# matsengrp/linearham

Hardware: AMD Instinct MI355X
Metric: phylo-HMM log-likelihood evals/sec (100-leaf x 400-site family) (higher is better)
Workload: dtype f64

## Files before the change

linearham_amd/csrc/lh_capi.hip:

```cpp
#include <algorithm>
#include <array>
#include <map>
#include <cstdio>
#include <cstring>
#include <functional>
#include <atomic>
#include <chrono>
#include <string>
#include <thread>
#include <utility>
#include <vector>

#include "lh_device.h"

namespace lh {
const DebugOptions& debug_options() {
  static const DebugOptions opts = [] {
    DebugOptions o;
    auto set = [](const char* name) { return std::getenv(name) != nullptr; };
    auto num = [](const char* name, int dflt) { const char* e = std::getenv(name); return e ? std::atoi(e) : dflt; };
    o.chunk = std::max(256, num("LH_CHUNK", o.chunk));
    o.host_sub = std::max(256, num("LH_HOST_SUB", o.host_sub));
    o.eval_split = std::min(8, std::max(0, num("LH_EVAL_SPLIT", o.eval_split)));
    o.k0_serial = set("LH_K0_SERIAL");
    o.eval_fwd_priority = std::min(1, num("LH_EVAL_FWD_PRIORITY", o.eval_fwd_priority));
    o.k2b_no_pair = set("LH_K2B_NO_PAIR");
    o.k2b_vd_single = set("LH_K2B_VD_SINGLE");
    o.k2b_dj_pair = set("LH_K2B_DJ_PAIR");
    o.sample_timing = set("LH_SAMPLE_TIMING");
    o.k4_no_save = set("LH_K4_NO_SAVE");
    o.k1_tile_cap = num("LH_K1_TILE_CAP", 0);
    o.k1_cxx_walk = set("LH_K1_CXX_WALK");
    o.k1_tables = set("LH_K1_TABLES");
    o.k1_stack = set("LH_K1_STACK");
    o.k1_no_tables = set("LH_K1_NO_TABLES");
    o.k1_segments = set("LH_K1_SEGMENTS");
    o.k1_seg_waves = num("LH_K1_SEG_WAVES", o.k1_seg_waves);
    o.k1_no_fuse = set("LH_K1_NO_FUSE");
    o.codon_blocks = std::max(1, num("LH_CODON_BLOCKS", o.codon_blocks));
    o.events_blocks = std::max(1, num("LH_EVENTS_BLOCKS", o.events_blocks));
    o.anc_out_mb = std::max(1, num("LH_ANC_OUT_MB", o.anc_out_mb));
    o.edge_out_mb = std::max(1, num("LH_EDGE_OUT_MB", o.edge_out_mb));
    o.anc_pairs = std::max(0, num("LH_ANC_PAIRS", o.anc_pairs));
    o.collect_hash_bits = std::min(64, std::max(1, num("LH_COLLECT_HASH_BITS", o.collect_hash_bits)));
    return o;
  }();
  return opts;
}
}

namespace {

thread_local std::string g_error;

int fail(const std::string& msg) {
  g_error = msg;
  return 1;
}

#define LH_HIP(expr)                                                                      \
  do {                                                                                    \
    hipError_t e_ = (expr);                                                               \
    if (e_ != hipSuccess)                                                                 \
      return fail(std::string(#expr) + ": " + hipGetErrorString(e_));                     \
  } while (0)

template <bool Pinned>
class Buffer {
 public:
  Buffer() = default;
  Buffer(const Buffer&) = delete;
  Buffer& operator=(const Buffer&) = delete;
  ~Buffer() { release(); }
  int ensure(size_t bytes) {
    bytes = std::max<size_t>(bytes, 64);
    if (bytes <= cap_) return 0;
    if (p_) {
      LH_HIP(hipDeviceSynchronize());
      release();
    }
    LH_HIP(Pinned ? hipHostMalloc(&p_, bytes, hipHostMallocDefault) : hipMalloc(&p_, bytes));
    cap_ = bytes;
    return 0;
  }
  template <typename T = void>
  T* get() const { return static_cast<T*>(p_); }

 private:
  void release() {
    if (p_) (void)(Pinned ? hipHostFree(p_) : hipFree(p_));
    p_ = nullptr;
    cap_ = 0;
  }
  void* p_ = nullptr;
  size_t cap_ = 0;
};
using DevBuf = Buffer<false>;
using PinnedBuf = Buffer<true>;

template <int Stages>
class KernelTimer {
 public:
  KernelTimer() = default;
  KernelTimer(const KernelTimer&) = delete;
  KernelTimer& operator=(const KernelTimer&) = delete;
  ~KernelTimer() {
    for (Events& es : done_) destroy(es);
    destroy(open_);
    destroy(done_spans_);
    destroy(open_spans_);
  }
  int begin(hipStream_t s) {
    destroy(open_);
    for (hipEvent_t& e : open_) LH_HIP(hipEventCreate(&e));
    return mark(0, s);
  }
  int mark(int k, hipStream_t s) {
    LH_HIP(hipEventRecord(open_[k], s));
    return 0;
  }
  int end(hipStream_t s) {
    if (mark(Stages, s)) return 1;
    done_.push_back(std::exchange(open_, Events{}));
    return 0;
  }
  void begin_spans() {
    destroy(open_);
    destroy(open_spans_);
  }
  int span_begin(int stage, hipStream_t s) {
    Span sp{stage, nullptr, nullptr};
    LH_HIP(hipEventCreate(&sp.a));
    open_spans_.push_back(sp);
    LH_HIP(hipEventCreate(&open_spans_.back().b));
    LH_HIP(hipEventRecord(sp.a, s));
    return 0;
  }
  int span_end(hipStream_t s) {
    LH_HIP(hipEventRecord(open_spans_.back().b, s));
    return 0;
  }
  void end_spans() {
    done_spans_.insert(done_spans_.end(), open_spans_.begin(), open_spans_.end());
    open_spans_.clear();
    ++span_groups_;
  }
  int read(double* ms, int64_t* launches) {
    double sum[Stages] = {};
    hipError_t e = hipSuccess;
    for (Span& sp : done_spans_) {
      if (e == hipSuccess) e = hipEventSynchronize(sp.b);
      float t = 0;
      if (e == hipSuccess) e = hipEventElapsedTime(&t, sp.a, sp.b);
      sum[sp.stage] += t;
    }
    destroy(done_spans_);
    for (Events& es : done_) {
      if (e == hipSuccess) e = hipEventSynchronize(es[Stages]);
      for (int k = 0; k < Stages && e == hipSuccess; ++k) {
        float t = 0;
        e = hipEventElapsedTime(&t, es[k], es[k + 1]);
        sum[k] += t;
      }
      destroy(es);
    }
    const int64_t n = (int64_t)done_.size() + std::exchange(span_groups_, 0);
    done_.clear();
    LH_HIP(e);
    if (ms) std::copy(sum, sum + Stages, ms);
    if (launches) *launches = n;
    return 0;
  }

 private:
  using Events = std::array<hipEvent_t, Stages + 1>;
  static void destroy(Events& es) {
    for (hipEvent_t& e : es)
// ... 3791 lines not shown
```

linearham_amd/csrc/lh_device.h:

```cpp
#pragma once
#include <hip/hip_runtime.h>
#include <stdint.h>

#include <functional>

#include "linearham_amd.h"

namespace lh {

constexpr double kScaleFactor = 0x1p256;
constexpr double kScaleThreshold = 0x1p-256;
constexpr double kLogScaleFactor = 177.445678223345993274;

template <class... P, class... A>
static inline void launch_lds(void (*kernel)(P...), dim3 grid, dim3 block, size_t lds, hipStream_t stream,
                              const A&... args) {
  if (lds > 64 * 1024)
    (void)hipFuncSetAttribute(reinterpret_cast<const void*>(kernel), hipFuncAttributeMaxDynamicSharedMemorySize, (int)lds);
  hipLaunchKernelGGL(kernel, grid, block, lds, stream, args...);
}

enum : int { OP_CHERRY = 0, OP_TIP_ACC = 1, OP_POP_ACC = 2, OP_PUSH_FLAG = 16, OP_RANK_SHIFT = 8 };

enum : int { W_CHERRY = 0, W_TIP_ACC = 1, W_POP = 2, W_CTIP = 3, W_CTAB_ACC = 4 };
// ... 209 lines not shown
  return b.anc + ((size_t)v * (b.T - 2) + (node - b.T)) * b.L;
}
__device__ inline const uint8_t* slot_row(const LineageBatch& b, int x) { return slot_row(b, x / (b.P + 1), x % (b.P + 1)); }
constexpr uint64_t kLineagePadHash = 0;
void launch_lineage(const LineageBatch& b, uint64_t* nt_hash, uint64_t* aa_hash, hipStream_t stream);

template <class Rows>
void launch_store_verify(const Rows& src, int K, const int32_t* ids, const uint8_t* store, uint8_t* flag,
                         hipStream_t stream);
template <class Rows>
void launch_store_append(const Rows& src, int K, int n_pairs, const int32_t* pairs, uint8_t* store, hipStream_t stream);
template <class Rows>
void launch_store_gather(const Rows& src, int n_out, const int32_t* slots, uint8_t* out, hipStream_t stream);

__device__ static inline void compute_pmatrix(const double* __restrict__ e, double tr, double P[4][4]) {
  double ex[4];
#pragma unroll
  for (int k = 1; k < 4; ++k) ex[k] = expm1(e[k] * tr);
#pragma unroll
  for (int i = 0; i < 4; ++i)
#pragma unroll
    for (int j = 0; j < 4; ++j) {
      double v = (i == j) ? 1.0 : 0.0;
#pragma unroll
      for (int k = 1; k < 4; ++k) v = fma(e[4 + i * 4 + k] * ex[k], e[20 + k * 4 + j], v);
      P[i][j] = fmax(v, 0.0);
    }
}


void launch_model_setup(int n, int R, const double* er, const double* pi, const double* alpha,
                        double* rates, double* eig, hipStream_t stream);

int launch_prune(const DevFamily& fam, int n, int R, int T, int max_depth, const int32_t* ops,
                 const double* brlen, const double* rates, const double* eig, const PruneWs& ws, const double* pi,
                 double* site_lik, int32_t* site_scal, hipStream_t stream, bool allow_fused = true,
                 bool test_every_op = false, const PruneFork* fork = nullptr);
const char* prune_last_form();
const char* prune_last_error();

void launch_gtr_setup(int n, const double* er, const double* pi, double* eig, hipStream_t stream);

int launch_asr(const DevFamily& fam, int n, int R, int T, const int32_t* ops, const double* brlen, const double* rates,
               const double* eig, const double* pi, const double* site_lik, const int32_t* site_scal,
               const uint8_t* naive, uint64_t seed, uint64_t sample0, double* clv, void* desc, uint8_t* anc,
               uint8_t* rate_choice, const int4* hdr , hipStream_t stream,
               int draws = 1);
size_t asr_desc_bytes(int T);
size_t asr_lds_bytes(int T, int L, int R, int n_prune);
size_t asr_slots(int L, int R);

struct AsrOp {
  int4 a, b;
};

void launch_asr_sched(int n, int T, const int32_t* ops, const int4* hdr, void* desc, hipStream_t stream);

struct AncWs {
  double* clv;
  double* part;
  double* tvec;
  double* rho;
  int32_t* chain;
  int32_t* plen;
  void* desc;
};
struct AncWsBytes {
  size_t clv, part, tvec, rho, chain;
  size_t total() const { return clv + part + tvec + rho + chain; }
};
AncWsBytes anc_ws_bytes(int T, int L, int R, int n_prune, int P);
size_t anc_lds_bytes(int T);
int launch_ancestral(const DevFamily& fam, int n, int R, int T, const int32_t* ops, const double* brlen, const double* rates,
                     const double* eig, const double* pi, const double* site_lik, const int32_t* site_scal,
                     const double* naive_prob, const int32_t* path, int P, const AncWs& ws, double* marg, double* rate_post,
                     const int4* hdr, int32_t* err_flag, hipStream_t stream);
void launch_site_base(int n, int L, size_t forward_size, const int32_t* off, const int32_t* idx, const double* post,
                      const double* loglik, double* site_base, hipStream_t stream);
void launch_ancestral_ends(int n, int P, int L, const int32_t* plen, const double* marg, const double* loglik, double* ends,
                           double* ll_used, hipStream_t stream);
void launch_ancestral_front(const DevFamily& fam, int n, int R, int T, const int32_t* ops, const double* pi,
                            const double* site_lik, const int32_t* site_scal, const double* naive_prob, const int32_t* path,
                            int P, const AncWs& ws, double* rate_post, const int4* hdr, int32_t* err_flag, hipStream_t stream);
size_t anc_lp(int n_prune);

void launch_rate_sum(int n, int R, int slots, size_t width, bool last_live, const int32_t* plen, const double* part,
                     double* out, hipStream_t stream);

struct SubWs {
  double* cc;
  double* ne;
  double* se;
  double* el;
  double* edge;
};
struct SubWsBytes {
  size_t cc, ne, se, el, edge;
  size_t total(bool with_edge) const { return cc + ne + se + el + (with_edge ? edge : 0); }
};
SubWsBytes sub_ws_bytes(int L, int R, int P);
size_t sub_lds_bytes(int T, int P);
struct SubOut {
  double *edge, *naive_edge, *chain_counts, *seed_edge, *edge_load, *rate_post;
};
int launch_substitutions(const DevFamily& fam, int n, int R, int T, const int32_t* ops, const double* brlen, const double* rates,
                         const double* eig, const double* pi, const double* site_lik, const int32_t* site_scal,
                         const double* naive_prob, const int32_t* path, int P, int seed_tip, const AncWs& ws, const SubWs& sws,
                         const SubOut& out, const int4* hdr, int32_t* err_flag, hipStream_t stream);

struct CondWsBytes {
  size_t part, table;
};
CondWsBytes cond_ws_bytes(int R, int n_prune);
int launch_ancestral_cond(const DevFamily& fam, int n, int R, int T, const int32_t* ops, const double* brlen,
                          const double* rates, const double* eig, const double* pi, const double* site_lik,
                          const int32_t* site_scal, const double* naive_prob, const int32_t* path, int P, int node,
                          const AncWs& ws, double* table, double* cond, const int4* hdr, int32_t* err_flag,
                          hipStream_t stream);
void launch_row_mask(int n, int C, const int32_t* plen, double* em, hipStream_t stream);
void launch_pair_emissions(const DevFamily& fam, int K, long long q0, int count, const uint8_t* seqs, const int32_t* col_site,
                           const uint8_t* col_base, const int32_t* plen, const double* em, const double* table, double* out,
                           hipStream_t stream);
void launch_pair_finish(int K, long long q0, int count, const double* pair_ll, const double* open_ll, const int32_t* plen,
                        double* log_cand, double* prob, hipStream_t stream);

struct LogEmRequest {
  const int32_t* cols = nullptr;
  int n = 0;
  double* out = nullptr;
};
void launch_forward(const DevFamily& fam, const DevFamily* fam_dev, int n, int R, const double* site_lik,
                    const int32_t* site_scal, const double* pi, const double* em_in, double* em_out, double* gem,
                    int32_t* gcnt, double* jem,
                    int32_t* jrs, double* dxf, int32_t* dxc, double* loglik, double* forward_out, int32_t* scaler_out,
                    bool extended, hipStream_t stream, const LogEmRequest& lem = LogEmRequest{});
size_t forward_lds_bytes(const DevFamily& fam);
const char* forward_last_form();
int forward_last_dj_samples();
int forward_last_dj_waves();

size_t viterbi_bp_bytes(const DevFamily& fam);
size_t viterbi_lds_bytes(const DevFamily& fam);
void launch_viterbi(const DevFamily& fam, const DevSampler* smp_dev, int n, const double* gem, const int32_t* gcnt,
                    const double* jem, const int32_t* jrs, const double* loglik, uint8_t* bp, int32_t* states,
                    double* log_path, bool extended, hipStream_t stream);
void launch_path_prior(const DevFamily& fam, const DevSampler* smp_dev, int K, const int32_t* states, double* log_prior,
                       int32_t* first_bad, hipStream_t stream);

struct DebugOptions {
  int chunk = 49152;
  int host_sub = 12288;
  int eval_split = 0;
  bool k0_serial = false;
  int eval_fwd_priority = -1;
  bool k2b_no_pair = false;
  bool k2b_vd_single = false;
  bool k2b_dj_pair = false;
  bool sample_timing = false;
  bool k4_no_save = false;
  int k1_tile_cap = 0;
  bool k1_cxx_walk = false;
  bool k1_tables = false;
  bool k1_stack = false;
  bool k1_no_tables = false;
  bool k1_segments = false;
  int k1_seg_waves = 4;
  bool k1_no_fuse = false;
  int codon_blocks = 2048;
  int events_blocks = 1024;
  int anc_out_mb = 4096;
  int edge_out_mb = 4096;
  int anc_pairs = 0;
  int collect_hash_bits = 64;
};
const DebugOptions& debug_options();

}
```

linearham_amd/csrc/lh_prune.hip:

```cpp
#include <cstdlib>

#include <cstdio>
#include <type_traits>

#include "lh_device.h"

namespace lh {

namespace {

thread_local char g_prune_form[64] = "";
thread_local char g_prune_error[256] = "";

#define LH_SLOT_COPY(dst, src)                       \
  _Pragma("unroll") for (int s_ = 0; s_ < S; ++s_) { \
    dst[s_][0] = src[s_][0];                         \
    dst[s_][1] = src[s_][1];                         \
    dst[s_][2] = src[s_][2];                         \
    dst[s_][3] = src[s_][3];                         \
  }
#define LH_PUSH_IF(d)                                   \
  if constexpr (kDepth > d) {                           \
    if (push_mask & (1u << d)) { LH_SLOT_COPY(st##d, a) } \
  }
// ... 554 lines not shown
          mat_list[rank] = (uint16_t)(2 * k);
          if (kind == OP_POP_ACC) mat_list[rank + 1] = (uint16_t)(2 * k + 1);
        }
      }
      __syncthreads();
      const int n_inner = T - 3;
      for (int it = rtid; it < n_inner + T; it += nthr) {
        if (it < n_inner) {
          const int code = mat_list[it], k = min(code >> 1, n_ops - 1);
          const int4 op = op_ptr[k];
          const int node = min(max((code & 1) ? op.y : op.z, 0), nodes - 1);
          compute_pmatrix(e, bl[node] * rt, P);
          double* o = pw + (size_t)k * 32 + (code & 1) * 16;
#pragma unroll
          for (int i = 0; i < 4; ++i)
#pragma unroll
            for (int q = 0; q < 4; ++q) o[i * 4 + q] = P[i][q];
        } else {
          const int j = it - n_inner;
          compute_pmatrix(e, bl[j] * rt, P);
          double* o = tiptab + j * 16;
#pragma unroll
          for (int i = 0; i < 4; ++i)
#pragma unroll
            for (int st = 0; st < 4; ++st) o[st * 4 + i] = P[i][st];
        }
      }
    } else {
    const int half = nthr >= 128 ? (nthr / 128) * 64 : 0;
    const bool do_ops = half == 0 || rtid < half;
    const bool do_tips = half == 0 || rtid >= half;
    if (do_ops) {
      const int stride = half ? half : nthr;
      for (int k = rtid; k < n_ops; k += stride) {
        const int4 op = op_ptr[k];
        const int kind = op.x & 15;
        if (kind == OP_CHERRY) continue;
        double* o = pw + (size_t)k * 32;
        compute_pmatrix(e, bl[op.z] * rt, P);
#pragma unroll
        for (int i = 0; i < 4; ++i)
#pragma unroll
          for (int q = 0; q < 4; ++q) o[i * 4 + q] = P[i][q];
        if (kind == OP_POP_ACC) {
          compute_pmatrix(e, bl[op.y] * rt, P);
#pragma unroll
          for (int i = 0; i < 4; ++i)
#pragma unroll
            for (int q = 0; q < 4; ++q) o[16 + i * 4 + q] = P[i][q];
        }
      }
    }
    if (do_tips) {
      const int stride = half ? nthr - half : nthr;
      for (int j = half ? rtid - half : rtid; j < (kSeg ? 1 : T); j += stride) {
        compute_pmatrix(e, bl[j] * rt, P);
        double* o = kSeg ? tiptab + 2 * kSegOps * 16 : tiptab + j * 16;
#pragma unroll
        for (int i = 0; i < 4; ++i)
#pragma unroll
          for (int st = 0; st < 4; ++st) o[st * 4 + i] = P[i][st];
      }
    }
    }
  }
  SegCtx seg{eig + (size_t)sample * 36, brlen + (size_t)sample * (2 * (size_t)T - 2),
             rates[(size_t)sample * R + rate], tiptab, rtid, nthr};
  if constexpr (kSeg) seg_fill(seg, op_ptr, n_ops, 0);
  asm volatile("s_waitcnt vmcnt(0)" ::: "memory");
  __threadfence_block();
  __syncthreads();

  const pmat_ptr pm = pmat_after_barrier(pmat_w + pm_off);
  const int lane = tid & 63;
  const int tile0 = blockIdx.x * tile;
  const int site_end = min(tile0 + tile, L);
  const double* __restrict__ p4 = pi + (size_t)sample * 4;
  double lik[2][5];
  int scl[2] = {0, 0};
  int site0, n_own;
  bool two_sites = false;
  if constexpr (kTwo) two_sites = wave < n2;
  if (two_sites) {
    site0 = tile0 + wave * 128 + lane;
    n_own = 2;
    if constexpr (kTwo)
      prune_wave<kDepth, 2, kN, kSeg>(site0, site_end, msa, L, n_ops, op_ptr, pm, tiptab, naive_tab, ones_off, p4, lik, scl, seg);
  } else {
    site0 = tile0 + n2 * 128 + (wave - n2) * 64 + lane;
    n_own = 1;
    double lik1[1][5];
    int scl1[1];
    prune_wave<kDepth, 1, kN, kSeg>(site0, site_end, msa, L, n_ops, op_ptr, pm, tiptab, naive_tab, ones_off, p4, lik1, scl1, seg);
#pragma unroll
    for (int b = 0; b < 5; ++b) lik[0][b] = lik1[0][b];
    scl[0] = scl1[0];
  }

  if constexpr (!kFused) {
    double* lik_out = site_lik + (((size_t)sample * R + rate) * 5) * (size_t)L;
    int32_t* scal_out = site_scal + ((size_t)sample * R + rate) * (size_t)L;
#pragma unroll
    for (int s = 0; s < 2; ++s) {
      const int site = site0 + 64 * s;
      if (s < n_own && site < site_end) {
#pragma unroll
        for (int b = 0; b < 5; ++b) lik_out[(size_t)b * L + site] = lik[s][b];
        scal_out[site] = scl[s];
      }
    }
  } else {
    const int pad = n2 * 128 + (wpr - n2) * 64;
    __syncthreads();
    double* X = reinterpret_cast<double*>(smem2);
    int* SC = reinterpret_cast<int*>(X + (size_t)R * 5 * pad);
#pragma unroll
    for (int s = 0; s < 2; ++s) {
      const int idx = site0 + 64 * s - tile0;
      if (s < n_own && idx < pad) {
#pragma unroll
        for (int b = 0; b < 5; ++b) X[((size_t)rate * 5 + b) * pad + idx] = lik[s][b];
        SC[rate * pad + idx] = scl[s];
      }
    }
    __syncthreads();
    const int n_tile = site_end - tile0;
    const double w = 1.0 / R;
    double* lik_out = site_lik + ((size_t)sample * 5) * (size_t)L;
    int32_t* scal_out = site_scal + (size_t)sample * (size_t)L;
    for (int j = tid; j < 5 * n_tile; j += blockDim.x) {
      const int b = j / n_tile, p = j - b * n_tile;
      int smin = 0x7fffffff;
      for (int r = 0; r < R; ++r) smin = min(smin, SC[r * pad + p]);
      double acc = 0.0;
      for (int r = 0; r < R; ++r) {
        double v = X[((size_t)r * 5 + b) * pad + p];
        const int d = SC[r * pad + p] - smin;
        for (int q = 0; q < d && v != 0.0; ++q) v *= kScaleThreshold;
        acc += w * v;
      }
      lik_out[(size_t)b * L + tile0 + p] = acc;
      if (b == 0) scal_out[tile0 + p] = smin;
    }
  }
}

__device__ __forceinline__ void matvec_v(const double (&p)[16], const double (&a)[4], double (&x)[4]) {
  x[0] = fma(p[3], a[3], fma(p[2], a[2], fma(p[1], a[1], p[0] * a[0])));
  x[1] = fma(p[7], a[3], fma(p[6], a[2], fma(p[5], a[1], p[4] * a[0])));
  x[2] = fma(p[11], a[3], fma(p[10], a[2], fma(p[9], a[1], p[8] * a[0])));
  x[3] = fma(p[15], a[3], fma(p[14], a[2], fma(p[13], a[1], p[12] * a[0])));
}

__global__ void __launch_bounds__(64) schedule_rewrite_kernel(int T, int max_depth, int tabs_stride, int use_tables,
                                                              const int32_t* __restrict__ ops, const double* __restrict__ brlen,
                                                              int2* __restrict__ wops, double* __restrict__ wlen,
                                                              int4* __restrict__ tabs, int4* __restrict__ hdr, int32_t* err_flag) {
  extern __shared__ int k0c_lds[];
  int* tnode = k0c_lds;
  int* lastpush = k0c_lds + tabs_stride;
  const int lane = threadIdx.x, smp = blockIdx.x;
  const int n_ops = T - 2, nodes = 2 * T - 2;
  const int4* __restrict__ og = reinterpret_cast<const int4*>(ops) + (size_t)smp * n_ops;
  int2* wo = wops + (size_t)smp * n_ops;
  int4* tl = tabs + (size_t)smp * tabs_stride;
  double* ml = wlen + (size_t)smp * n_ops;
  const double* __restrict__ bl = brlen + (size_t)smp * nodes;
  if (lane < 16) lastpush[lane] = -1;
  __syncthreads();
  auto tip_ok = [&](int v) { return v >= 1 && v < T; };
  auto inner_ok = [&](int v) { return v >= T && v < nodes; };
  auto plain = [](int x) { return x >= 0 && (x & 0xf0) == 0; };
  auto fold = [&](int j, const int4& c, const int4& nx) -> int {
    if (!use_tables || j + 1 >= n_ops || (c.x & 15) != OP_CHERRY || c.x < 0 || (c.x & 0xe0)) return 0;
    const bool push = (c.x & OP_PUSH_FLAG) != 0;
    const int nk = nx.x & 15;
    if (push && nk == OP_POP_ACC && plain(nx.x) && nx.w == c.w && inner_ok(nx.y) && inner_ok(nx.z)) return 1;
    if (nk == OP_TIP_ACC && plain(nx.x) && tip_ok(nx.y) && inner_ok(nx.z)) return 2;
    return 0;
  };
  auto scan = [&](int v) {
#pragma unroll
    for (int d = 1; d < 64; d <<= 1) {
      const int up = __shfl_up(v, d);
      if (lane >= d) v += up;
    }
    return v;
  };
  int c_bdepth = 0, c_wi = 0, c_wdepth = 0, c_mi = 0, c_ti = 0;
  bool bad = false;
  const int4 none = make_int4(15, 0, 0, 0);
  for (int k0 = 0; k0 < n_ops; k0 += 64) {
    const int k = k0 + lane;
    const bool in = k < n_ops;
    const int4 op = in ? og[k] : none;
    const int4 nx = (in && k + 1 < n_ops) ? og[k + 1] : none;
    const int4 pv = (in && k > 0) ? og[k - 1] : none;
    const int kind = op.x & 15;
    const bool push = (op.x & OP_PUSH_FLAG) != 0;
    const int f = in ? fold(k, op, nx) : 0;
    const bool consumed = in && k > 0 && fold(k - 1, pv, op) != 0;
    bool ok = op.x >= 0 && (op.x & 0xe0) == 0 && kind <= OP_POP_ACC;
    if (kind == OP_CHERRY) ok = ok && tip_ok(op.y) && tip_ok(op.z) && push == (k != 0);
    if (kind == OP_TIP_ACC) ok = ok && !push && k > 0 && tip_ok(op.y) && inner_ok(op.z);
    if (kind == OP_POP_ACC) ok = ok && !push && k > 0 && inner_ok(op.y) && inner_ok(op.z);
    const int db = !in || !ok ? 0 : push ? 1 : kind == OP_POP_ACC ? -1 : 0;
    const int s_db = scan(db);
    const int bdepth = c_bdepth + s_db - db;
    if (in && push && (op.w != bdepth || bdepth >= max_depth)) ok = false;
    if (in && kind == OP_POP_ACC && op.w != bdepth - 1) ok = false;
    const bool emit = in && ok && !consumed;
    const bool wpush = emit && push && f != 1;
    const bool wpop = emit && kind == OP_POP_ACC;
    const bool hasmat = wpush || (emit && (f == 1 || kind == OP_TIP_ACC || kind == OP_POP_ACC));
    const bool hastab = emit && f != 0;
    const int e1 = emit ? 1 : 0, dw = wpush ? 1 : wpop ? -1 : 0, m1 = hasmat ? 1 : 0, t1 = hastab ? 1 : 0;
    const int s_e1 = scan(e1), s_dw = scan(dw), s_m1 = scan(m1), s_t1 = scan(t1);
    const int wi = c_wi + s_e1 - e1, wdepth = c_wdepth + s_dw - dw, mi = c_mi + s_m1 - m1, ti = c_ti + s_t1 - t1;
    if (wpush && wdepth >= 16) ok = false;
    if (wpop && wdepth < 1) ok = false;
    if (hastab && ti >= tabs_stride) ok = false;
    if (hasmat && mi >= n_ops) ok = false;
    if (in && !ok) bad = true;
    int mypush = -1;
    for (int d = 0; d < max_depth; ++d) {
      int v = (wpush && ok && wdepth == d) ? mi : -1;
#pragma unroll
      for (int q = 1; q < 64; q <<= 1) {
        const int up = __shfl_up(v, q);
        if (lane >= q) v = max(v, up);
      }
      v = max(v, lastpush[d]);
      if (wpop && wdepth - 1 == d) mypush = v;
      const int last = __shfl(v, 63);
      __syncthreads();
      if (lane == 0) lastpush[d] = last;
      __syncthreads();
    }
    if (wpop && mypush < 0) {
      ok = false;
      bad = true;
    }
    if (emit && ok) {
      int2 w;
      if (f == 1) {
        w = make_int2(W_CTAB_ACC | WOP_MATRIX | WOP_HAS_B | (op.y << 16), op.z | (1 << 16));
        ml[mi] = bl[nx.y];
      } else if (kind == OP_CHERRY) {
        const int pushbits = wpush ? WOP_MATRIX | ((wdepth + 1) << WOP_PUSH_SHIFT) : 0;
        w = f == 2 ? make_int2(W_CTIP | pushbits | WOP_HAS_B | WOP_HAS_C | (op.y << 16), op.z | (nx.y << 16))
                   : make_int2(W_CHERRY | pushbits | WOP_HAS_B | (op.y << 16), op.z | (1 << 16));
      } else if (kind == OP_TIP_ACC) {
        w = make_int2(W_TIP_ACC | WOP_MATRIX | (op.y << 16), 1 | (1 << 16));
        ml[mi] = bl[op.z];
      } else {
        w = make_int2(W_POP | WOP_MATRIX | ((wdepth - 1) << WOP_POP_SHIFT) | (1 << 16), 1 | (1 << 16));
        ml[mypush] = bl[op.y];
        ml[mi] = bl[op.z];
      }
      wo[wi] = w;
      if (hastab) {
        tl[ti] = make_int4(op.y, op.z, nx.z, 0);
        tnode[ti] = nx.z;
      }
    }
    c_bdepth += __shfl(s_db, 63);
    c_wi += __shfl(s_e1, 63);
    c_wdepth += __shfl(s_dw, 63);
    c_mi += __shfl(s_m1, 63);
    c_ti += __shfl(s_t1, 63);
  }
  if (c_bdepth != 0 || c_wdepth != 0 || c_mi + c_ti > T - 3) bad = true;
  const bool any_bad = __builtin_amdgcn_ballot_w64(bad) != 0;
  if (lane == 0) {
    if (any_bad) {
      hdr[smp] = make_int4(0, 0, 0, 1);
      atomicOr(err_flag, 1);
    } else {
      hdr[smp] = make_int4(c_wi, c_mi, c_ti, 0);
    }
  }
  if (any_bad) return;
  __syncthreads();
  for (int c = lane; c < c_ti; c += 64) ml[c_mi + c] = bl[tnode[c]];
}

__global__ void __launch_bounds__(64) schedule_stack_check_kernel(int T, int slots, int check_ranks,
                                                                  const int32_t* __restrict__ ops, int4* __restrict__ hdr,
                                                                  int32_t* err_flag) {
  const int smp = blockIdx.x, lane = threadIdx.x;
  const int n_ops = T - 2, nodes = 2 * T - 2;
  const int4* __restrict__ o = reinterpret_cast<const int4*>(ops) + (size_t)smp * n_ops;
  int carry = 0, depth0 = 0;
  bool bad = false;
  for (int k0 = 0; k0 < n_ops; k0 += 64) {
    const int k = k0 + lane;
    const bool in = k < n_ops;
    const int4 op = in ? o[k] : make_int4(OP_CHERRY, 1, 1, 0);
    const int kind = op.x & 15, rank = op.x >> OP_RANK_SHIFT;
    const bool push = (op.x & OP_PUSH_FLAG) != 0;
    bool ok = op.x >= 0 && (op.x & 0xe0) == 0 && kind <= OP_POP_ACC;
    if (kind == OP_CHERRY) ok = ok && op.y >= 1 && op.y < T && op.z >= 1 && op.z < T && push == (k != 0);
    if (kind == OP_TIP_ACC) ok = ok && !push && k > 0 && op.y >= 1 && op.y < T && op.z >= T && op.z < nodes;
    if (kind == OP_POP_ACC) ok = ok && !push && k > 0 && op.y >= T && op.y < nodes && op.z >= T && op.z < nodes;
    if (push || kind == OP_POP_ACC) ok = ok && op.w >= 0 && op.w < slots;
    const int m = !in || !ok ? 0 : kind == OP_TIP_ACC ? 1 : kind == OP_POP_ACC ? 2 : 0;
    const int dl = !in || !ok ? 0 : push ? 1 : kind == OP_POP_ACC ? -1 : 0;
    int incl = m, dincl = dl;
#pragma unroll
    for (int d = 1; d < 64; d <<= 1) {
      const int up = __shfl_up(incl, d), dup = __shfl_up(dincl, d);
      if (lane >= d) incl += up, dincl += dup;
    }
    const int depth = depth0 + dincl - dl;
    if (in && push && op.w != depth) ok = false;
    if (in && kind == OP_POP_ACC && op.w != depth - 1) ok = false;
    if (check_ranks && in && kind != OP_CHERRY && rank != carry + incl - m) ok = false;
    if (in && !ok) bad = true;
    carry += __shfl(incl, 63);
    depth0 += __shfl(dincl, 63);
  }
  if (carry != T - 3 || depth0 != 0) bad = true;
  const bool any_bad = __builtin_amdgcn_ballot_w64(bad) != 0;
  if (lane == 0) {
    hdr[smp] = make_int4(0, 0, 0, any_bad ? 1 : 0);
    if (any_bad) atomicOr(err_flag, 1);
  }
}

struct PruneCtArgs {
  int n2, tile, R, wpr;
  int L, T, tabs_stride, pad_;
  const uint8_t* msa;
  const uint64_t* planes;
  const int2* wops;
  const double* wlen;
  const int4* tabs;
  const int4* hdr;
  const double* brlen;
  const double* rates;
  const double* eig;
  double* pmat_w;
  size_t rate_stride;
  const double* pi;
  double* site_lik;
  int32_t* site_scal;
};
typedef const PruneCtArgs __attribute__((address_space(4)))* ct_args_ptr;
typedef int __attribute__((ext_vector_type(4))) ct_int4;

__device__ __forceinline__ ct_args_ptr ct_args_again(ct_args_ptr p) {
  uint64_t v = reinterpret_cast<uint64_t>(p);
  asm volatile("; lh: kernel arguments at %0, read again from here" : "+s"(v));
  return (ct_args_ptr)v;
}
__device__ __forceinline__ ct_args_ptr ct_args() { return ct_args_again((ct_args_ptr)__builtin_amdgcn_kernarg_segment_ptr()); }

template <class T, class U>
__device__ __forceinline__ const T __attribute__((address_space(4)))* ct_ro(const U* p) {
  return (const T __attribute__((address_space(4)))*)reinterpret_cast<uint64_t>(p);
}

struct CtWave {
  int rate, wave, nthr, rtid;
};
constexpr int kCtFusedMaxWaves = 16;
constexpr size_t kCtFusedMaxLds = 80 * 1024;
static_assert(kCtFusedMaxWaves <= 16, "ct_wave counts at most 15 steps");
static_assert(53 * 1024 <= kCtFusedMaxLds, "the limit of fused workgroups of up to eight waves (launch_prune) lies within it");
static_assert(3 * (kCtFusedMaxLds / 128) < (1u << 21), "prune_body_ct: c / rem through v_rcp_f32 needs R * rem < 2^21");
template <bool kFused>
__device__ __forceinline__ int ct_block_threads(int R, int wpr) {
  return (kFused ? R : 1) * wpr * 64;
}
template <bool kFused>
__device__ __forceinline__ CtWave ct_wave(int tid, int wpr) {
  const int wave_all = __builtin_amdgcn_readfirstlane(tid >> 6);
  if constexpr (kFused) {
    int rate = 0, wave = wave_all;
    for (; wave >= wpr && rate < 15; ++rate) wave -= wpr;
    return CtWave{rate, wave, wpr * 64, tid - rate * wpr * 64};
  } else {
    return CtWave{(int)blockIdx.y, wave_all, wpr * 64, tid};
  }
}

template <int kDepth, bool kN, bool kFused, bool kAsm = false>
__device__ __forceinline__ void prune_body_ct() {
  extern __shared__ double2 smem2[];
  constexpr int SY = kN ? 5 : 4, E = SY * SY;
  constexpr int kS = 2;
  const int tid = threadIdx.x;
  const int sample = blockIdx.z;
  const ct_args_ptr a0 = ct_args();
  const CtWave g = ct_wave<kFused>(tid, a0->wpr);
  const int rate = g.rate, wave = g.wave, nthr = g.nthr, rtid = g.rtid;
  {
    const ct_args_ptr a = a0;
    const int T = a->T, R = a->R;
    const int n_w = ct_ro<int>(a->hdr)[(size_t)sample * 4];
    if (kN && tid < 4) reinterpret_cast<double*>(smem2)[(kFused ? R : 1) * T * 16 + tid] = 1.0;
    const WalkOp* wops = a->wops + (size_t)sample * (T - 2);
    WalkOp* desc = reinterpret_cast<WalkOp*>(reinterpret_cast<double*>(smem2) + (size_t)(kFused ? R : 1) * T * 16 + (kN ? 4 : 0));
    for (int i = tid; i < n_w; i += ct_block_threads<kFused>(R, a->wpr))
      desc[i] = *reinterpret_cast<const WalkOp*>(reinterpret_cast<const char*>(wops) + (unsigned)i * 8u);
  }

  int4 tcell = make_int4(1, 1, 0, 0);
  double pcq[16];
  {
    const ct_args_ptr a = a0;
    const int T = a->T, R = a->R, n_ops = T - 2;
    const int n_mat = ct_ro<int>(a->hdr)[(size_t)sample * 4 + 1], n_tab = ct_ro<int>(a->hdr)[(size_t)sample * 4 + 2];
    const size_t rate_stride = a->rate_stride;
    const int n_q = min(n_tab, nthr >> 2);
    const bool in_quad = (rtid >> 2) < n_q;
    const bool pc_lane = (rtid & 3) == 0 && in_quad;
    if (in_quad) tcell = (a->tabs + (size_t)sample * a->tabs_stride)[rtid >> 2];
    const double* bl = a->brlen + (size_t)sample * (2 * (size_t)T - 2);
    const double* wl = a->wlen + (size_t)sample * n_ops;
    char* pw_s = reinterpret_cast<char*>(a->pmat_w + (size_t)sample * R * rate_stride);
    const unsigned rate_bytes = (unsigned)rate_stride * 8u;
    const int n_rest = n_tab - n_q;
// ... 204 lines not shown
    for (int s = 0; s < kS; ++s) {
      const int site = site0 + 64 * s;
      if (s < n_own && site < site_end) {
#pragma unroll
        for (int q = 0; q < 5; ++q) lik_out[(size_t)q * L_b + site] = lik[s][q];
        scal_out[site] = scl[s];
      }
    }
  } else {
    const int pad = n2_b * (64 * kS) + (b->wpr - n2_b) * 64;
    __syncthreads();
    double* X = reinterpret_cast<double*>(smem2);
    int* SC = reinterpret_cast<int*>(X + (size_t)R_b * 5 * pad);
#pragma unroll
    for (int s = 0; s < kS; ++s) {
      const int idx = site0 + 64 * s - tile0;
      if (s < n_own && idx < pad) {
#pragma unroll
        for (int q = 0; q < 5; ++q) X[((size_t)rate_b * 5 + q) * pad + idx] = lik[s][q];
        SC[rate_b * pad + idx] = scl[s];
      }
    }
    __syncthreads();
    const int n_tile = site_end - tile0;
    const double w = 1.0 / R_b;
    double* lik_out = b->site_lik + ((size_t)sample * 5) * (size_t)L_b;
    int32_t* scal_out = b->site_scal + (size_t)sample * (size_t)L_b;
    for (int p = tid_b; p < n_tile; p += ct_block_threads<kFused>(R_b, b->wpr)) {
      int smin = 0x7fffffff;
      for (int r = 0; r < R_b; ++r) smin = min(smin, SC[r * pad + p]);
      double acc[5] = {0.0, 0.0, 0.0, 0.0, 0.0};
      for (int r = 0; r < R_b; ++r) {
        const int d = SC[r * pad + p] - smin;
#pragma unroll
        for (int q = 0; q < 5; ++q) {
          double v = X[((size_t)r * 5 + q) * pad + p];
          for (int k = 0; k < d && v != 0.0; ++k) v *= kScaleThreshold;
          acc[q] += w * v;
        }
      }
#pragma unroll
      for (int q = 0; q < 5; ++q) lik_out[(size_t)q * L_b + tile0 + p] = acc[q];
      scal_out[tile0 + p] = smin;
    }
  }
}

#define LH_PRUNE_CT_KERNEL(NAME, WAVES)                                                              \
  template <int kDepth, bool kN, bool kFused, bool kAsm>                                             \
  __global__ void __launch_bounds__(1024) __attribute__((amdgpu_waves_per_eu(WAVES, WAVES))) NAME(   \
      const PruneCtArgs args ) {                                         \
    prune_body_ct<kDepth, kN, kFused, kAsm>();                                                       \
  }
LH_PRUNE_CT_KERNEL(prune_kernel_ct6, 6)
LH_PRUNE_CT_KERNEL(prune_kernel_ct5, 5)
LH_PRUNE_CT_KERNEL(prune_kernel_ct4, 4)
#undef LH_PRUNE_CT_KERNEL
#define LH_PRUNE_PARAMS                                                                                     \
  int n_samples, int n2, int tile, int R, int wpr, const uint8_t *__restrict__ msa, int L, int T, int n_ops, \
      const int32_t *__restrict__ ops, const int4 *__restrict__ hdr, int32_t *err_flag,                     \
      const double *__restrict__ brlen, const double *__restrict__ rates, const double *__restrict__ eig,  \
      double *pmat_w, size_t rate_stride, const double *__restrict__ pi,                                   \
      double *__restrict__ site_lik, int32_t *__restrict__ site_scal
#define LH_PRUNE_ARGS \
  n2, tile, R, wpr, msa, L, T, n_ops, ops, hdr, err_flag, brlen, rates, eig, pmat_w, rate_stride, pi, site_lik, site_scal
#define LH_PRUNE_SAMPLES(BODY) BODY((int)blockIdx.z, LH_PRUNE_ARGS);

#define LH_PRUNE_KERNEL(NAME, WAVES)                                                                 \
  template <int kDepth, bool kN>                                                                     \
  __global__ void __launch_bounds__(1024) __attribute__((amdgpu_waves_per_eu(WAVES, WAVES))) NAME(   \
      LH_PRUNE_PARAMS) {                                                                             \
    LH_PRUNE_SAMPLES((prune_body<kDepth, true, kN, true>))                                           \
  }
LH_PRUNE_KERNEL(prune_kernel_w6, 6)
LH_PRUNE_KERNEL(prune_kernel_w5, 5)
LH_PRUNE_KERNEL(prune_kernel_w4, 4)
#undef LH_PRUNE_KERNEL

template <int kDepth, bool kN>
__global__ void __launch_bounds__(512) __attribute__((amdgpu_waves_per_eu(5, 5))) prune_kernel_seg(LH_PRUNE_PARAMS) {
  LH_PRUNE_SAMPLES((prune_body<kDepth, true, kN, false, true>))
}
template <int kDepth, bool kN>
__global__ void __launch_bounds__(512) __attribute__((amdgpu_waves_per_eu(4, 4))) prune_kernel_seg4(LH_PRUNE_PARAMS) {
  LH_PRUNE_SAMPLES((prune_body<kDepth, true, kN, false, true>))
}

PruneWsSizes prune_ws_sizes(int T, bool mixed_n) {
  PruneWsSizes z;
  z.tabs_per_sample = (size_t)std::max((T - 1) / 2, 1);
  const size_t e = mixed_n ? 25 : 16;
  z.scratch_doubles_per_rate = std::max((size_t)std::max(T - 3, 0) * 16 + z.tabs_per_sample * e * 4, (size_t)std::max(T - 2, 1) * 32);
  return z;
}

int launch_prune(const DevFamily& fam, int n, int R, int T, int max_depth, const int32_t* ops,
                 const double* brlen, const double* rates, const double* eig, const PruneWs& ws, const double* pi,
                 double* site_lik, int32_t* site_scal, hipStream_t stream, bool allow_fused, bool test_every_op,
                 const PruneFork* fork) {
  hipStream_t sched = fork ? fork->sched : stream;
  auto joined = [&]() {
    if (!fork || fork->join() == 0) return true;
    snprintf(g_prune_error, sizeof(g_prune_error), "K1: the schedule kernel's stream could not be joined");
    return false;
  };
  const int L = fam.n_prune;
  const PruneWsSizes sizes = prune_ws_sizes(T, fam.msa_mixed_n != 0);
  if (L == 0) {
    hipLaunchKernelGGL(schedule_stack_check_kernel, dim3(n), dim3(64), 0, sched, T, std::max(max_depth, 1), 0, ops, ws.hdr, ws.err_flag);
    return joined() ? R : -1;
  }
  double* pmat = ws.scratch;
  const size_t rate_stride = sizes.scratch_doubles_per_rate;
  const DebugOptions& dbg = debug_options();
  const int cap_env = dbg.k1_tile_cap;
  const int cap = cap_env >= 64 ? std::min(cap_env, 1024) : 1024;
  const int tiles = (L + cap - 1) / cap;
  const int tile = tiles == 1 ? L : (((L + tiles - 1) / tiles + 127) & ~127);
  int n2 = tile / 128, n1;
  {
    const int rem = tile - 128 * n2;
    if (rem > 64) {
      ++n2;
      n1 = 0;
    } else {
      n1 = rem > 0 ? 1 : 0;
    }
  }
  const int wpr = n2 + n1;
  const size_t tip_bytes = (size_t)T * 16 * sizeof(double);
  const size_t pad = (size_t)n2 * 128 + (size_t)n1 * 64;
  const size_t tail_bytes = (((size_t)std::max(T - 2, 1) * sizeof(int2)) + 31) & ~(size_t)15;
  const bool mixed = fam.msa_mixed_n != 0;
  const size_t ones_bytes = mixed ? 32 : 0;
  const size_t fused_lds = std::max((size_t)R * tip_bytes + ones_bytes + tail_bytes, (size_t)R * pad * (5 * sizeof(double) + sizeof(int)));
  const bool fused = allow_fused && !dbg.k1_no_fuse && !dbg.k1_segments &&
                     ((R * wpr <= 8 && fused_lds <= 53 * 1024) ||
                      (R * wpr > 8 && R * wpr <= kCtFusedMaxWaves && fused_lds <= kCtFusedMaxLds));
  const bool big = !fused && ((160 * 1024 / tip_bytes) * wpr / 4 < 5 || dbg.k1_segments);
  const bool tables_hook = dbg.k1_tables || dbg.k1_no_tables;
  const bool use_asm = !dbg.k1_cxx_walk && !test_every_op;
  const bool stack_fused = fused && max_depth <= 4 && dbg.k1_stack && !tables_hook;
  const bool seg = big && max_depth <= 4 && !tables_hook;
  const size_t seg_bytes = (size_t)(2 * kSegOps + 1) * 16 * sizeof(double) + ones_bytes;
  size_t lds = fused ? fused_lds : seg ? seg_bytes : tip_bytes + ones_bytes + tail_bytes;
  if (lds > 160 * 1024) {
    snprintf(g_prune_error, sizeof(g_prune_error),
             "K1: a tree of %d tips with stack depth %d needs %zu bytes of LDS in the cherry-table form (160 KB per CU)", T, max_depth, lds);
    return -1;
  }
  if (stack_fused || seg) {
    hipLaunchKernelGGL(schedule_stack_check_kernel, dim3(n), dim3(64), 0, sched, T, stack_fused && max_depth <= 3 ? 3 : 4,
                       stack_fused ? 1 : 0, ops, ws.hdr, ws.err_flag);
  } else {
    hipLaunchKernelGGL(schedule_rewrite_kernel, dim3(n), dim3(64), (sizes.tabs_per_sample + 16) * sizeof(int), sched, T, max_depth,
                       (int)sizes.tabs_per_sample, dbg.k1_no_tables ? 0 : 1, ops, brlen, ws.wops, ws.wlen, ws.tabs, ws.hdr, ws.err_flag);
  }
  if (!joined()) return -1;
  const int wg_waves = fused ? R * wpr : wpr;
  dim3 grid(tiles, fused ? 1 : R, n), block(64 * wg_waves);
  const int n_ops = T - 2;
  hipError_t attr_rc = hipSuccess;
#define LH_LAUNCH_K(K, NAME)                                                                                     \
  {                                                                                                              \
    if (lds > 64 * 1024)                                                                                         \
      attr_rc = hipFuncSetAttribute(reinterpret_cast<const void*>(K), hipFuncAttributeMaxDynamicSharedMemorySize, (int)lds); \
    snprintf(g_prune_form, sizeof(g_prune_form), "%s", NAME);                                                    \
    if (attr_rc == hipSuccess)                                                                                   \
      hipLaunchKernelGGL(K, grid, block, lds, stream, n, n2, tile, R, wpr, fam.msa, L, T, n_ops, ops, ws.hdr, ws.err_flag, \
                         brlen, rates, eig, pmat, rate_stride, pi, site_lik, site_scal);                        \
  }
#define LH_LAUNCH_CT(K, NAME)                                                                                    \
  {                                                                                                              \
    if (lds > 64 * 1024)                                                                                         \
      attr_rc = hipFuncSetAttribute(reinterpret_cast<const void*>(K), hipFuncAttributeMaxDynamicSharedMemorySize, (int)lds); \
    snprintf(g_prune_form, sizeof(g_prune_form), "%s", NAME);                                                    \
    if (attr_rc == hipSuccess) hipLaunchKernelGGL(K, grid, block, lds, stream, ct_args);                        \
  }
  PruneCtArgs ct_args = {};
  ct_args.n2 = n2, ct_args.tile = tile, ct_args.R = R, ct_args.wpr = wpr;
  ct_args.L = L, ct_args.T = T, ct_args.tabs_stride = (int)sizes.tabs_per_sample;
  ct_args.msa = fam.msa, ct_args.planes = fam.msa_planes;
  ct_args.wops = ws.wops, ct_args.wlen = ws.wlen, ct_args.tabs = ws.tabs, ct_args.hdr = ws.hdr;
  ct_args.brlen = brlen, ct_args.rates = rates, ct_args.eig = eig;
  ct_args.pmat_w = pmat, ct_args.rate_stride = rate_stride;
  ct_args.pi = pi, ct_args.site_lik = site_lik, ct_args.site_scal = site_scal;
  const int lds_waves = lds == 0 ? 8 : (int)((160 * 1024 / lds) * wg_waves / 4);
  if (stack_fused) {
#define LH_LAUNCH_STACK(D, N)                                                          \
  {                                                                                    \
    if (lds_waves >= 6 && D == 3)                                                      \
      LH_LAUNCH_K((prune_kernel_w6<D, N>), "w6<" #D "," #N ">")                        \
    else if (lds_waves >= 5)                                                           \
      LH_LAUNCH_K((prune_kernel_w5<D, N>), "w5<" #D "," #N ">")                        \
    else                                                                               \
      LH_LAUNCH_K((prune_kernel_w4<D, N>), "w4<" #D "," #N ">")                        \
  }
    if (max_depth <= 3 && !mixed)
      LH_LAUNCH_STACK(3, false)
    else if (max_depth <= 3)
      LH_LAUNCH_STACK(3, true)
    else if (!mixed)
      LH_LAUNCH_STACK(4, false)
    else
      LH_LAUNCH_STACK(4, true)
#undef LH_LAUNCH_STACK
  } else if (seg) {
    if (dbg.k1_seg_waves == 4) {
      if (mixed)
        LH_LAUNCH_K((prune_kernel_seg4<4, true>), "seg4<4,true>")
      else
        LH_LAUNCH_K((prune_kernel_seg4<4, false>), "seg4<4,false>")
    } else {
      if (mixed)
        LH_LAUNCH_K((prune_kernel_seg<4, true>), "seg5<4,true>")
      else
        LH_LAUNCH_K((prune_kernel_seg<4, false>), "seg5<4,false>")
    }
  } else {
#define LH_LAUNCH_BUDGET(D, N, F, A)                                                          \
  {                                                                                           \
    if (lds_waves >= 6)                                                                       \
      LH_LAUNCH_CT((prune_kernel_ct6<D, N, F, A>), "ct6<" #D "," #N "," #F "," #A ">")        \
    else if (lds_waves >= 5)                                                                  \
      LH_LAUNCH_CT((prune_kernel_ct5<D, N, F, A>), "ct5<" #D "," #N "," #F "," #A ">")        \
    else                                                                                      \
      LH_LAUNCH_CT((prune_kernel_ct4<D, N, F, A>), "ct4<" #D "," #N "," #F "," #A ">")        \
  }
#define LH_LAUNCH_FORM(D, N, A)        \
  {                                    \
    if (fused)                         \
      LH_LAUNCH_BUDGET(D, N, true, A)  \
    else                               \
      LH_LAUNCH_BUDGET(D, N, false, A) \
  }
#define LH_LAUNCH_SHALLOW(D)           \
  {                                    \
    if (mixed && use_asm)              \
      LH_LAUNCH_FORM(D, true, true)    \
    else if (mixed)                    \
      LH_LAUNCH_FORM(D, true, false)   \
    else if (use_asm)                  \
      LH_LAUNCH_FORM(D, false, true)   \
    else                               \
      LH_LAUNCH_FORM(D, false, false)  \
  }
    if (max_depth <= 4)
      LH_LAUNCH_SHALLOW(4)
    else
      LH_LAUNCH_SHALLOW(16)
#undef LH_LAUNCH_SHALLOW
#undef LH_LAUNCH_FORM
#undef LH_LAUNCH_BUDGET
  }
#undef LH_LAUNCH_K
#undef LH_LAUNCH_CT
  const hipError_t launch_rc = attr_rc == hipSuccess ? hipGetLastError() : attr_rc;
  if (launch_rc != hipSuccess) {
    snprintf(g_prune_error, sizeof(g_prune_error), "K1 launch (%s, %zu bytes of LDS): %s", g_prune_form, lds, hipGetErrorString(launch_rc));
    return -1;
  }
  return fused ? 1 : R;
}

const char* prune_last_form() { return g_prune_form; }
const char* prune_last_error() { return g_prune_error; }

}
```

Before: 8.774 million.

## Rewrite schedule-rewrite kernel scans with DPP and register-held stack state

The schedule rewrite kernel (K0c) now does its wave-wide prefix scans with DPP row and broadcast operations instead of shfl_up loops. The four count scans are packed into one 32-bit word so a single scan covers them. The per-depth last-push table moves from LDS into a register read with readlane, which removes two barriers per depth level. Neighbour ops now come from lane shifts instead of extra global loads. The old shfl path stays behind an environment flag; the new path relies on exact DPP row-mask semantics and on packed fields not overflowing.

```diff
diff --git a/linearham_amd/csrc/lh_capi.hip b/linearham_amd/csrc/lh_capi.hip
--- a/linearham_amd/csrc/lh_capi.hip
+++ b/linearham_amd/csrc/lh_capi.hip
@@ -23,6 +23,7 @@
     o.host_sub = std::max(256, num("LH_HOST_SUB", o.host_sub));
     o.eval_split = std::min(8, std::max(0, num("LH_EVAL_SPLIT", o.eval_split)));
     o.k0_serial = set("LH_K0_SERIAL");
+    o.k0c_shfl = set("LH_K0C_SHFL");
     o.eval_fwd_priority = std::min(1, num("LH_EVAL_FWD_PRIORITY", o.eval_fwd_priority));
     o.k2b_no_pair = set("LH_K2B_NO_PAIR");
     o.k2b_vd_single = set("LH_K2B_VD_SINGLE");
diff --git a/linearham_amd/csrc/lh_device.h b/linearham_amd/csrc/lh_device.h
--- a/linearham_amd/csrc/lh_device.h
+++ b/linearham_amd/csrc/lh_device.h
@@ -385,6 +385,7 @@
   int host_sub = 12288;
   int eval_split = 0;
   bool k0_serial = false;
+  bool k0c_shfl = false;
   int eval_fwd_priority = -1;
   bool k2b_no_pair = false;
   bool k2b_vd_single = false;
diff --git a/linearham_amd/csrc/lh_prune.hip b/linearham_amd/csrc/lh_prune.hip
--- a/linearham_amd/csrc/lh_prune.hip
+++ b/linearham_amd/csrc/lh_prune.hip
@@ -730,6 +730,48 @@
   x[3] = fma(p[15], a[3], fma(p[14], a[2], fma(p[13], a[1], p[12] * a[0])));
 }
 
+template <int kCtrl, int kRowMask>
+__device__ __forceinline__ int dpp_or_zero(int v) {
+  return __builtin_amdgcn_update_dpp(0, v, kCtrl, kRowMask, 0xf, false);
+}
+__device__ __forceinline__ int next_lane(int v) { return dpp_or_zero<0x130, 0xf>(v); }
+__device__ __forceinline__ int prev_lane(int v) { return dpp_or_zero<0x138, 0xf>(v); }
+template <int kN, typename Op>
+__device__ __forceinline__ void wave_scan(int (&v)[kN], Op op) {
+#pragma unroll
+  for (int i = 0; i < kN; ++i) v[i] = op(v[i], dpp_or_zero<0x111, 0xf>(v[i]));
+#pragma unroll
+  for (int i = 0; i < kN; ++i) v[i] = op(v[i], dpp_or_zero<0x112, 0xf>(v[i]));
+#pragma unroll
+  for (int i = 0; i < kN; ++i) v[i] = op(v[i], dpp_or_zero<0x114, 0xf>(v[i]));
+#pragma unroll
+  for (int i = 0; i < kN; ++i) v[i] = op(v[i], dpp_or_zero<0x118, 0xf>(v[i]));
+#pragma unroll
+  for (int i = 0; i < kN; ++i) v[i] = op(v[i], dpp_or_zero<0x142, 0xa>(v[i]));
+#pragma unroll
+  for (int i = 0; i < kN; ++i) v[i] = op(v[i], dpp_or_zero<0x143, 0xc>(v[i]));
+}
+__device__ __forceinline__ int wave_scan_add(int x) {
+  int v[1] = {x};
+  wave_scan(v, [](int a, int b) { return a + b; });
+  asm("" : "+v"(v[0]));
+  return v[0];
+}
+template <int kN>
+__device__ __forceinline__ void wave_scan_umax(int (&v)[kN]) {
+  wave_scan(v, [](int a, int b) { return (int)max((unsigned)a, (unsigned)b); });
+}
+
+struct K0cPacked {
+  static constexpr int kCountBits = 7, kDepthBits = 8;
+  static constexpr int kM1 = kCountBits, kT1 = 2 * kCountBits, kDw = 3 * kCountBits;
+  static constexpr unsigned kCountMask = (1u << kCountBits) - 1;
+  static_assert(64 * 1 <= kCountMask, "a count over 64 lanes must fit its field");
+  static_assert(64 * 2 <= (1u << kDepthBits) - 1, "the biased depth change (0/1/2) over 64 lanes must fit its field");
+  static_assert(kDw + kDepthBits <= 32, "four fields in one word");
+};
+
+template <bool kShfl>
 __global__ void __launch_bounds__(64) schedule_rewrite_kernel(int T, int max_depth, int tabs_stride, int use_tables,
                                                               const int32_t* __restrict__ ops, const double* __restrict__ brlen,
                                                               int2* __restrict__ wops, double* __restrict__ wlen,
@@ -744,8 +786,11 @@
   int4* tl = tabs + (size_t)smp * tabs_stride;
   double* ml = wlen + (size_t)smp * n_ops;
   const double* __restrict__ bl = brlen + (size_t)smp * nodes;
-  if (lane < 16) lastpush[lane] = -1;
-  __syncthreads();
+  if constexpr (kShfl) {
+    if (lane < 16) lastpush[lane] = -1;
+    __syncthreads();
+  }
+  unsigned lastpush_r = 0;
   auto tip_ok = [&](int v) { return v >= 1 && v < T; };
   auto inner_ok = [&](int v) { return v >= T && v < nodes; };
   auto plain = [](int x) { return x >= 0 && (x & 0xf0) == 0; };
@@ -758,26 +803,47 @@
     return 0;
   };
   auto scan = [&](int v) {
-#pragma unroll
-    for (int d = 1; d < 64; d <<= 1) {
-      const int up = __shfl_up(v, d);
-      if (lane >= d) v += up;
-    }
-    return v;
+    if constexpr (!kShfl) {
+      return wave_scan_add(v);
+    } else {
+#pragma unroll
+      for (int d = 1; d < 64; d <<= 1) {
+        const int up = __shfl_up(v, d);
+        if (lane >= d) v += up;
+      }
+      return v;
+    }
   };
   int c_bdepth = 0, c_wi = 0, c_wdepth = 0, c_mi = 0, c_ti = 0;
+  int c_f = 0;
   bool bad = false;
   const int4 none = make_int4(15, 0, 0, 0);
   for (int k0 = 0; k0 < n_ops; k0 += 64) {
     const int k = k0 + lane;
     const bool in = k < n_ops;
-    const int4 op = in ? og[k] : none;
-    const int4 nx = (in && k + 1 < n_ops) ? og[k + 1] : none;
-    const int4 pv = (in && k > 0) ? og[k - 1] : none;
+    int4 op, nx;
+    int f;
+    bool consumed;
+    if constexpr (kShfl) {
+      op = in ? og[k] : none;
+      nx = (in && k + 1 < n_ops) ? og[k + 1] : none;
+      const int4 pv = (in && k > 0) ? og[k - 1] : none;
+      f = in ? fold(k, op, nx) : 0;
+      consumed = in && k > 0 && fold(k - 1, pv, op) != 0;
+    } else {
+      const int4 raw = og[min(k, n_ops - 1)];
+      op = in ? raw : none;
+      int4 far = none;
+      if (lane == 63 && k + 1 < n_ops) far = og[k + 1];
+      nx = make_int4(next_lane(op.x), next_lane(op.y), next_lane(op.z), next_lane(op.w));
+      if (lane == 63) nx = far;
+      f = in ? fold(k, op, nx) : 0;
+      const int f_prev = prev_lane(f);
+      consumed = in && (lane == 0 ? c_f : f_prev) != 0;
+      c_f = __builtin_amdgcn_readlane(f, 63);
+    }
     const int kind = op.x & 15;
     const bool push = (op.x & OP_PUSH_FLAG) != 0;
-    const int f = in ? fold(k, op, nx) : 0;
-    const bool consumed = in && k > 0 && fold(k - 1, pv, op) != 0;
     bool ok = op.x >= 0 && (op.x & 0xe0) == 0 && kind <= OP_POP_ACC;
     if (kind == OP_CHERRY) ok = ok && tip_ok(op.y) && tip_ok(op.z) && push == (k != 0);
     if (kind == OP_TIP_ACC) ok = ok && !push && k > 0 && tip_ok(op.y) && inner_ok(op.z);
@@ -793,7 +859,16 @@
     const bool hasmat = wpush || (emit && (f == 1 || kind == OP_TIP_ACC || kind == OP_POP_ACC));
     const bool hastab = emit && f != 0;
     const int e1 = emit ? 1 : 0, dw = wpush ? 1 : wpop ? -1 : 0, m1 = hasmat ? 1 : 0, t1 = hastab ? 1 : 0;
-    const int s_e1 = scan(e1), s_dw = scan(dw), s_m1 = scan(m1), s_t1 = scan(t1);
+    int s_e1, s_dw, s_m1, s_t1;
+    unsigned s_packed = 0;
+    if constexpr (kShfl) {
+      s_e1 = scan(e1), s_dw = scan(dw), s_m1 = scan(m1), s_t1 = scan(t1);
+    } else {
+      using P = K0cPacked;
+      s_packed = (unsigned)wave_scan_add(e1 | (m1 << P::kM1) | (t1 << P::kT1) | ((dw + 1) << P::kDw));
+      s_e1 = s_packed & P::kCountMask, s_m1 = (s_packed >> P::kM1) & P::kCountMask, s_t1 = (s_packed >> P::kT1) & P::kCountMask;
+      s_dw = (int)(s_packed >> P::kDw) - (lane + 1);
+    }
     const int wi = c_wi + s_e1 - e1, wdepth = c_wdepth + s_dw - dw, mi = c_mi + s_m1 - m1, ti = c_ti + s_t1 - t1;
     if (wpush && wdepth >= 16) ok = false;
     if (wpop && wdepth < 1) ok = false;
@@ -801,19 +876,44 @@
     if (hasmat && mi >= n_ops) ok = false;
     if (in && !ok) bad = true;
     int mypush = -1;
-    for (int d = 0; d < max_depth; ++d) {
-      int v = (wpush && ok && wdepth == d) ? mi : -1;
-#pragma unroll
-      for (int q = 1; q < 64; q <<= 1) {
-        const int up = __shfl_up(v, q);
-        if (lane >= q) v = max(v, up);
-      }
-      v = max(v, lastpush[d]);
-      if (wpop && wdepth - 1 == d) mypush = v;
-      const int last = __shfl(v, 63);
-      __syncthreads();
-      if (lane == 0) lastpush[d] = last;
-      __syncthreads();
+    if constexpr (kShfl) {
+      for (int d = 0; d < max_depth; ++d) {
+        int v = (wpush && ok && wdepth == d) ? mi : -1;
+#pragma unroll
+        for (int q = 1; q < 64; q <<= 1) {
+          const int up = __shfl_up(v, q);
+          if (lane >= q) v = max(v, up);
+        }
+        v = max(v, lastpush[d]);
+        if (wpop && wdepth - 1 == d) mypush = v;
+        const int last = __shfl(v, 63);
+        __syncthreads();
+        if (lane == 0) lastpush[d] = last;
+        __syncthreads();
+      }
+    } else {
+      const int pushlvl = (wpush && ok) ? wdepth : -1, poplvl = wpop ? wdepth - 1 : -1;
+      const int slot1 = mi + 1;
+      unsigned found = 0;
+      for (int d0 = 0; d0 < max_depth; d0 += 2) {
+        int lvl[2], v[2];
+        unsigned before[2];
+#pragma unroll
+        for (int j = 0; j < 2; ++j) {
+          lvl[j] = d0 + j < max_depth ? d0 + j : INT_MIN;
+          v[j] = pushlvl == lvl[j] ? slot1 : 0;
+          before[j] = (unsigned)__builtin_amdgcn_readlane((int)lastpush_r, d0 + j);
+        }
+        wave_scan_umax(v);
+#pragma unroll
+        for (int j = 0; j < 2; ++j) {
+          const unsigned u = max((unsigned)v[j], before[j]);
+          if (poplvl == lvl[j]) found = u;
+          const unsigned last = (unsigned)__builtin_amdgcn_readlane((int)u, 63);
+          if (lane == d0 + j) lastpush_r = last;
+        }
+      }
+      mypush = (int)found - 1;
     }
     if (wpop && mypush < 0) {
       ok = false;
@@ -842,11 +942,21 @@
         tnode[ti] = nx.z;
       }
     }
-    c_bdepth += __shfl(s_db, 63);
-    c_wi += __shfl(s_e1, 63);
-    c_wdepth += __shfl(s_dw, 63);
-    c_mi += __shfl(s_m1, 63);
-    c_ti += __shfl(s_t1, 63);
+    if constexpr (kShfl) {
+      c_bdepth += __shfl(s_db, 63);
+      c_wi += __shfl(s_e1, 63);
+      c_wdepth += __shfl(s_dw, 63);
+      c_mi += __shfl(s_m1, 63);
+      c_ti += __shfl(s_t1, 63);
+    } else {
+      using P = K0cPacked;
+      const unsigned tot = (unsigned)__builtin_amdgcn_readlane((int)s_packed, 63);
+      c_bdepth += __builtin_amdgcn_readlane(s_db, 63);
+      c_wi += tot & P::kCountMask;
+      c_mi += (tot >> P::kM1) & P::kCountMask;
+      c_ti += (tot >> P::kT1) & P::kCountMask;
+      c_wdepth += (int)(tot >> P::kDw) - 64;
+    }
   }
   if (c_bdepth != 0 || c_wdepth != 0 || c_mi + c_ti > T - 3) bad = true;
   const bool any_bad = __builtin_amdgcn_ballot_w64(bad) != 0;
@@ -1357,8 +1467,11 @@
   if (stack_fused || seg) {
     hipLaunchKernelGGL(schedule_stack_check_kernel, dim3(n), dim3(64), 0, sched, T, stack_fused && max_depth <= 3 ? 3 : 4,
                        stack_fused ? 1 : 0, ops, ws.hdr, ws.err_flag);
+  } else if (dbg.k0c_shfl) {
+    hipLaunchKernelGGL(schedule_rewrite_kernel<true>, dim3(n), dim3(64), (sizes.tabs_per_sample + 16) * sizeof(int), sched, T, max_depth,
+                       (int)sizes.tabs_per_sample, dbg.k1_no_tables ? 0 : 1, ops, brlen, ws.wops, ws.wlen, ws.tabs, ws.hdr, ws.err_flag);
   } else {
-    hipLaunchKernelGGL(schedule_rewrite_kernel, dim3(n), dim3(64), (sizes.tabs_per_sample + 16) * sizeof(int), sched, T, max_depth,
+    hipLaunchKernelGGL(schedule_rewrite_kernel<false>, dim3(n), dim3(64), sizes.tabs_per_sample * sizeof(int), sched, T, max_depth,
                        (int)sizes.tabs_per_sample, dbg.k1_no_tables ? 0 : 1, ops, brlen, ws.wops, ws.wlen, ws.tabs, ws.hdr, ws.err_flag);
   }
   if (!joined()) return -1;
```

Measured after the change: 8.838 million (median of 6 runs). Within noise of the previous version (+0.7%).
